# longliangLiu/PriOr-Flow

Measured on AMD Instinct MI355X. Metric: frame-pairs/sec @512x1024 iters=12; EPE vs reference, higher is better.
Workload: dtype bf16x3 split MFMA, f32 accumulate/storage; 1 GPU; PriOr-RAFT forward, 1 synthetic 512x1024 ERP pair(s) per GPU per step, iters=12, test_mode (BASELINE.json configs[1]); height=512, width=1024, iters=12, parallelism=pairs sharded over 1 rank(s), no data-path collective, weights=deterministic closed-form fill (no checkpoints offline), hip_graph=True, encoders=libpriorflow_hip.so (HIP kernels, both precisions)

## Files before the change

### __graft_entry__.py

```python
from __future__ import annotations

import os
import shutil
import subprocess
import sys

ROOT = os.path.dirname(os.path.abspath(__file__))
PKG = os.path.join(ROOT, "prior-flow_amd")
CSRC = os.path.join(PKG, "csrc")
LIB_DIR = os.path.join(PKG, "lib")
LIB = os.path.join(LIB_DIR, "libpriorflow_hip.so")
HIP_UNITS = [("pf_elem_kernels.hip", [], "pf_elem_kernels"), ("pf_lookup.hip", [], "pf_lookup"),
             ("pf_conv_mfma.hip", ["-DPF_CONV_PART=0"], "pf_conv_mfma.p0"), ("pf_conv_mfma.hip", ["-DPF_CONV_PART=1"], "pf_conv_mfma.p1"),
             ("pf_conv_mfma.hip", ["-DPF_CONV_PART=2"], "pf_conv_mfma.p2"), ("pf_conv_mfma.hip", ["-DPF_CONV_PART=3"], "pf_conv_mfma.p3"),
             ("pf_conv_mfma.hip", ["-DPF_CONV_PART=4"], "pf_conv_mfma.p4"),
             ("pf_conv_api.hip", [], "pf_conv_api"),
             ("pf_corr_mfma.hip", [], "pf_corr_mfma"), ("pf_enc_stem.hip", [], "pf_enc_stem"), ("pf_enc_conv.hip", [], "pf_enc_conv"), ("pf_flow_stem.hip", [], "pf_flow_stem"), ("pf_corr_conv.hip", [], "pf_corr_conv"), ("pf_conv_bwd.hip", [], "pf_conv_bwd"),
             ("pf_augment.hip", [], "pf_augment")]
HIP_UNITS += [("pf_conv_dma.hip", [f"-DPF_DMA_PART={i}"], f"pf_conv_dma.p{i}") for i in (0, 1, 2, 3, 4, 5, 6, 7, 8, 9)]
HIP_SOURCES = sorted({u[0] for u in HIP_UNITS})
HIP_DEPS = ["pf_common.h", "pf_elem.h", "pf_split.h", "pf_conv_priv.h", "pf_api_elem.inc", os.path.join("..", "..", "include", "priorflow_hip.h")]
HIPCC_FLAGS = ["--offload-arch=gfx950", "-O3", "-ffp-contract=off", "-fno-slp-vectorize", "-fPIC", "-shared"]


def _stale(target: str, sources) -> bool:
    if not os.path.exists(target):
        return True
    t = os.path.getmtime(target)
    return any(os.path.getmtime(s) > t for s in sources if os.path.exists(s))


def _deps_of(dfile: str, fallback):
    try:
        txt = open(dfile).read().replace("\\\n", " ")
# ... 127 lines not shown
```

### prior-flow_amd/csrc/pf_conv_api.hip

```cpp
#include <stdlib.h>
#include "pf_conv_priv.h"

using namespace pfconv;

static int conv_prepare(const pf_conv_desc* descs, int ngroups, int B, int H8, int W8,
                        ConvGroups& grp, ConvGeom& g, int& max_cout) {
    if (!descs || ngroups < 1 || ngroups > MAX_GROUPS) return PF_ERR_BAD_ARG;
    if (B <= 0 || H8 <= 0 || W8 <= 0) return PF_ERR_BAD_SHAPE;
    max_cout = 0;
    const pf_conv_desc& f = descs[0];
    for (int i = 0; i < ngroups; ++i) {
        const pf_conv_desc& d = descs[i];
        if ((!d.in0 && !d.in0_split) || !d.weight || !d.bias || (!d.out && !d.out_split)) return PF_ERR_BAD_ARG;
        if (d.c0 <= 0 || d.c1 < 0 || (d.c1 > 0 && !d.in1 && !d.in1_split)) return PF_ERR_BAD_ARG;
        const bool f16 = d.precision == PF_PREC_F16;
        const int cpc = f16 ? 64 : 32, cm = cpc - 1;
        if ((d.in0_split || d.in1_split || d.out_split || d.aux_split) && d.precision != PF_PREC_BF16X3 && !f16) return PF_ERR_BAD_ARG;
        if (f16 && (!d.in0_split || (d.c1 > 0 && !d.in1_split))) return PF_ERR_BAD_ARG;
        if (d.in0_split && ((d.off0 & cm) || d.lds0 * cpc < d.off0 + d.c0)) return PF_ERR_BAD_SHAPE;
        if (d.in1_split && d.c1 > 0 && ((d.off1 & cm) || (d.c0 & cm) || d.lds1 * cpc < d.off1 + d.c1)) return PF_ERR_BAD_SHAPE;
        if (d.in0_split && d.c1 == 0 && (d.c0 & cm) && d.off0 + ((d.c0 + cm) & ~cm) != d.lds0 * cpc) return PF_ERR_BAD_SHAPE;
        if (d.in1_split && d.c1 > 0 && (d.c1 & cm) && d.off1 + ((d.c1 + cm) & ~cm) != d.lds1 * cpc) return PF_ERR_BAD_SHAPE;
        if (d.out_split && ((d.off_out & 31) || d.lds_out <= 0)) return PF_ERR_BAD_SHAPE;
        if (d.aux_split && d.lds_aux * cpc < 128) return PF_ERR_BAD_SHAPE;
// ... 58 lines not shown
static bool roles_apply(const ConvGroups& grp, int ngroups, const ConvGeom& g) {
    if (!((g.kh == 3 && g.kw == 3) || (g.kh == 1 && g.kw == 5) || (g.kh == 5 && g.kw == 1)) || g.stride != 1) return false;
    for (int i = 0; i < ngroups; ++i)
        if (grp.d[i].stats_out != nullptr || grp.d[i].in_scale != nullptr) return false;
    return true;
}

static int conv_dma_choice(const ConvGroups& grp, int ngroups, const ConvGeom& g, int max_cout, int tile_id) {
    if (!grp.d[0].in0_split || tile_id < 3 || tile_id == 7 || !roles_apply(grp, ngroups, g)) return 0;
    if (tile_id == 5) return 2;
    const long wgs256 = (long)(g.M / g.N) * ((g.H + 7) / 8) * ((g.W + 31) / 32) * (ngroups + grp.d[0].co_groups) * ((max_cout + 63) / 64);
    if (g.kh != 3 && max_cout > 128 && wgs256 >= 256) return 2;
    return (g.kh == 3 && max_cout > 64 && wgs256 >= 256) ? 2 : 1;
}

static int conv_ws_choice(const ConvGroups& grp, int ngroups, const ConvGeom& g, int max_cout) {
    static const int ws = [] { const char* e = getenv("PRIORFLOW_CONV_WS"); return e ? atoi(e) : 2; }();
    if (ws <= 0 || !roles_apply(grp, ngroups, g)) return 0;
    const long wgs256 = (long)(g.M / g.N) * ((g.H + 7) / 8) * ((g.W + 31) / 32) * ngroups * ((max_cout + 63) / 64);
    if (ws >= 3 && g.kh == 3 && wgs256 >= 256) return 2;
    return (ws >= 2 && g.kh == 3 && max_cout > 64 && wgs256 >= 256) ? 2 : 1;
}

static int conv_plan(const pf_conv_desc* descs, int ngroups, int B, int H8, int W8, ConvPlan& p) {
    if (const int rc = conv_prepare(descs, ngroups, B, H8, W8, p.grp, p.g, p.max_cout)) return rc;
    const ConvGroups& grp = p.grp;
    const ConvGeom& g = p.g;
    p.ngroups = ngroups;
    p.tile = conv_tile(g, ngroups + descs[0].co_groups, p.max_cout, descs[0].precision);
    const int dma = conv_dma_choice(grp, ngroups, g, p.max_cout, p.tile);
    if (descs[0].precision == PF_PREC_F16 && !dma) return PF_ERR_BAD_SHAPE;
    const bool split = descs[0].precision == PF_PREC_BF16X3;
    const bool generic = p.tile < 3 || p.tile == 7;
    const int bm = (p.tile == 0 || p.tile == 7) ? 128 : 64;
    for (int i = 0; i < ngroups; ++i) {
        if (descs[i].in_scale && generic) return PF_ERR_BAD_SHAPE;
        if (descs[i].stats_out && descs[i].epilogue != PF_EPI_LINEAR) return PF_ERR_BAD_SHAPE;
        if (descs[i].stats_out && generic && (!split || g.N % bm != 0)) return PF_ERR_BAD_SHAPE;
    }
    const bool enc64 = (p.tile == 5 || p.tile == 3) && pf_enc_conv64_applies(grp, ngroups, g, p.max_cout);
    const int th = (p.tile == 5 || p.tile == 8) ? 8 : 4;
    p.stats_blocks = enc64 ? pf_enc_conv64_stats_blocks(g)
                   : generic ? ((split && g.N % bm == 0) ? g.N / bm : 0) : ((g.H + th - 1) / th) * ((g.W + 31) / 32);
    p.affine = false;
    if (dma) {
        for (int i = 0; i < ngroups; ++i)
            if (!descs[i].zeros || descs[i].zeros_bytes < 128 * (descs[i].lds0 > descs[i].lds1 ? descs[i].lds0 : descs[i].lds1)) return PF_ERR_BAD_ARG;
        p.roles = 16 + dma;
        p.launch = dma == 2 ? pf_conv_dma_launch<2, 1> : p.tile == 4 ? pf_conv_dma_launch<2, 2> : pf_conv_dma_launch<1, 2>;
        return PF_OK;
    }
    for (int i = 0; i < ngroups; ++i) {
        if (!descs[i].in0 || (descs[i].c1 > 0 && !descs[i].in1)) return PF_ERR_BAD_ARG;
        if (descs[i].pre) return PF_ERR_BAD_SHAPE;
    }
    p.roles = 0;
    if (enc64) { p.tile = 6; p.launch = pf_enc_conv64_launch; return PF_OK; }
    if (!generic) {
        p.affine = descs[0].in_scale != nullptr;
        for (int i = 1; i < ngroups; ++i)
            if ((descs[i].in_scale != nullptr) != p.affine) return PF_ERR_BAD_ARG;
        if (p.affine && (g.kh != 3 || g.kw != 3)) return PF_ERR_BAD_SHAPE;
    }
    if (p.tile == 3 || p.tile == 4) p.roles = conv_ws_choice(grp, ngroups, g, p.max_cout);
// ... 37 lines not shown
```

### prior-flow_amd/csrc/pf_conv_dma.hip

```cpp
#include <stdlib.h>
#include "pf_conv_priv.h"

namespace {
using namespace pfconv;

template <int HP, int HSTEPS>
constexpr int hbeg_(int t) { return t >= HSTEPS ? HP : HP * t / HSTEPS; }

template <int N>
__device__ __forceinline__ void wait_vmcnt() {
#if defined(__HIP_DEVICE_COMPILE__)
    asm volatile("s_waitcnt vmcnt(%0)" :: "n"(N) : "memory");
#endif
}
__device__ __forceinline__ void wg_barrier() {
#if defined(__HIP_DEVICE_COMPILE__) && !defined(PF_DMA_ABL_NO_BARRIER)
    asm volatile("s_barrier" ::: "memory");
#endif
}

struct DmaItem { int grp, tile, ntile; };


typedef _Float16 f16x8 __attribute__((ext_vector_type(8)));

template <int NT, int KH, int KW, int WN, bool F16>
__global__ void __launch_bounds__(512, 2)
pf_conv_dma_kernel(const ConvGroups groups, const ConvGeom g) {
    static_assert(WN == 1 || WN == 2, "");
    constexpr int TH = 8 / WN, TW = 32, BN = 32 * NT * WN, TAPS = KH * KW;
    static_assert(TAPS >= 5, "the halo schedule needs TAPS - 3 >= 2 issue steps");
    constexpr int HW = TW + KW - 1, HH = TH + KH - 1;
    constexpr int HP = (HH * HW + 31) / 32;
    constexpr int HALO_ROWS = 32 * HP, HALO_BYTES = HALO_ROWS * 128;
    constexpr int WP = BN / 32;
    constexpr int SLOT_BYTES = BN * 128;
    constexpr int HSTEPS = TAPS - 3;
    constexpr int CSH = F16 ? 6 : 5;
    extern __shared__ __attribute__((aligned(128))) char smem[];
    constexpr int RING = 2 * HALO_BYTES;

    const int tid = threadIdx.x;
    const int lane = tid & 63, wave = __builtin_amdgcn_readfirstlane(tid >> 6);
    const int li = lane & 31, lh = lane >> 5;
    const int tiles_x = (g.W + TW - 1) / TW, tiles_y = (g.H + TH - 1) / TH;
// ... 151 lines not shown
                        if (ih) wait_vmcnt<hp + WP + hc>();
                        else wait_vmcnt<WP>();
                    } else {
                        wait_vmcnt<0>();
                    }
                    slot3 = (slot3 + 1) & 3;
                });
            }
            have = have_next;
            if (have) have_next = next_item(j, nit);
        }
        return;
    }

    const int wy2 = WN == 2 ? wave >> 1 : wave, wn = WN == 2 ? wave & 1 : 0;
    f32x16 acc[2][NT];
    const unsigned arow0 = (unsigned)((2 * wy2) * HW + li);
    const unsigned P0 = 2u * lh;
    const unsigned b_off = (unsigned)(32 * NT * wn + li) * 128 + ((P0 ^ (((unsigned)(32 * NT * wn + li) >> 1) & 7u)) << 4);
    bf16x8 fa[2][2][4], fb[2][NT][4];
#ifdef PF_DMA_ABL_NO_READS
    for (int i = 0; i < 2; ++i)
        for (int k = 0; k < 4; ++k) {
            for (int m = 0; m < 2; ++m) for (int e = 0; e < 8; ++e) fa[i][m][k][e] = (__bf16)(float)(lane & 7);
            for (int t = 0; t < NT; ++t) for (int e = 0; e < 8; ++e) fb[i][t][k][e] = (__bf16)(float)(lane & 3);
        }
#endif
    unsigned a_addr[2] = {0, 0}, b_addr = 0;
    unsigned a_base[TAPS][2];
    auto set_a_base = [&]() __attribute__((always_inline)) {
        unsigned ar = arow0;
#if defined(__HIP_DEVICE_COMPILE__)
        asm volatile("" : "+v"(ar));
#endif
#pragma unroll
        for (int tp = 0; tp < TAPS; ++tp)
#pragma unroll
            for (int m = 0; m < 2; ++m) {
                const unsigned hr = ar + (unsigned)((tp / KW + m) * HW + tp % KW);
                a_base[tp][m] = (hr << 7) + ((P0 ^ ((hr >> 1) & 7u)) << 4);
            }
    };
    set_a_base();
    constexpr int NP = 8 + 4 * NT;
    constexpr int NM = (F16 ? 8 : 12) * NT;
    constexpr int FETCH_GAPS = NM - 2;
    auto fetch_piece = [&](auto SET, auto P, unsigned halo_off, auto TAP, unsigned slot_off) __attribute__((always_inline)) {
        constexpr int set = decltype(SET)::value, p = decltype(P)::value, tp = decltype(TAP)::value;
        if constexpr (p < 8) {
            constexpr int m = p / 4, k = p % 4;
            if constexpr (k == 0) {
                unsigned a0 = halo_off + a_base[tp][m];
#if defined(__HIP_DEVICE_COMPILE__)
                asm volatile("" : "+v"(a0));
#endif
                a_addr[m] = a0;
            }
            constexpr unsigned x = (k & 1) * 16u + (k >> 1) * 64u;
#ifndef PF_DMA_ABL_NO_READS
            fa[set][m][k] = *reinterpret_cast<const bf16x8*>(smem + (a_addr[m] ^ x));
#endif
        } else {
            constexpr int t = (p - 8) / 4, k = (p - 8) % 4;
            if constexpr (t == 0 && k == 0) b_addr = (unsigned)RING + slot_off + b_off;
            constexpr unsigned x = (k & 1) * 16u + (k >> 1) * 64u;
#ifndef PF_DMA_ABL_NO_READS
            fb[set][t][k] = *reinterpret_cast<const bf16x8*>(smem + (b_addr ^ x) + t * 4096);
#endif
        }
    };
    unsigned jm = wslot;
    DmaItem it;
    if (!next_item(jm, it)) return;
    wg_barrier();
    static_for<0, NP>([&](auto P) __attribute__((always_inline)) { fetch_piece(std::integral_constant<int, 0>{}, P, 0u, std::integral_constant<int, 0>{}, 0u); });
    int slot1 = 1;
    int gc = 0;
    auto mstep = [&](auto U) __attribute__((always_inline)) {
        constexpr int u = decltype(U)::value;
        constexpr int tap = u % TAPS, cur = u & 1;
        constexpr int ntap = (tap + 1) % TAPS;
        const unsigned halo_off = (unsigned)(((tap == TAPS - 1 ? gc + 1 : gc) & 1) * HALO_BYTES), slot_off = (unsigned)(slot1 * SLOT_BYTES);
        using NXT = std::integral_constant<int, cur ^ 1>;
        wg_barrier();
        static_for<0, NM>([&](auto I) __attribute__((always_inline)) {
            constexpr int i = decltype(I)::value;
            constexpr int idx = i % (2 * NT), m = idx / NT, t = idx % NT, j = i / (2 * NT), ks = j / 3, pass = j % 3;
#ifdef PF_DMA_ABL_NO_MFMA
            if constexpr (F16)
                asm volatile("" :: "v"(fa[cur][m][j]), "v"(fb[cur][t][j]));
            else if constexpr (pass == 0)
                asm volatile("" :: "v"(fa[cur][m][ks]), "v"(fa[cur][m][2 + ks]), "v"(fb[cur][t][ks]), "v"(fb[cur][t][2 + ks]));
#else
            if constexpr (F16)
                acc[m][t] = __builtin_amdgcn_mfma_f32_32x32x16_f16(__builtin_bit_cast(f16x8, fa[cur][m][j]),
                                                                  __builtin_bit_cast(f16x8, fb[cur][t][j]), acc[m][t], 0, 0, 0);
            else if constexpr (pass == 0)
                acc[m][t] = __builtin_amdgcn_mfma_f32_32x32x16_bf16(fa[cur][m][2 + ks], fb[cur][t][ks], acc[m][t], 0, 0, 0);
            else if constexpr (pass == 1)
                acc[m][t] = __builtin_amdgcn_mfma_f32_32x32x16_bf16(fa[cur][m][ks], fb[cur][t][2 + ks], acc[m][t], 0, 0, 0);
            else
                acc[m][t] = __builtin_amdgcn_mfma_f32_32x32x16_bf16(fa[cur][m][ks], fb[cur][t][ks], acc[m][t], 0, 0, 0);
// ... 6 lines not shown
        });
        slot1 = (slot1 + 1) & 3;
        if constexpr (tap == TAPS - 1) ++gc;
    };
    const bool ragged = (g.W % TW) != 0 || (g.H % TH) != 0;
    bool have = true;
    while (have) {
        if (const float* pre = gdesc[it.grp].pre) {
            const auto& dp = gdesc[it.grp];
            const int ldp = dp.ld_pre, jb = it.ntile * BN + 32 * NT * wn + li;
            const int cout = dp.cout;
            pre += dp.off_pre;
            int x0, y0; long pix0;
            tile_origin(it, x0, y0, pix0);
#pragma unroll
            for (int m = 0; m < 2; ++m) {
                const int wy = 2 * wy2 + m;
                const int xlim = (y0 + wy < g.H) ? g.W - x0 - 4 * lh : 0;
                const long pm = pix0 + (long)(y0 + wy) * g.W + x0 + 4 * lh;
#pragma unroll
                for (int t = 0; t < NT; ++t) {
                    const bool jok = jb + 32 * t < cout;
                    const float* pp = pre + pm * ldp + jb + 32 * t;
#pragma unroll
                    for (int r = 0; r < 16; ++r) {
                        const int ro = (r & 3) + 8 * (r >> 2);
                        acc[m][t][r] = (jok && ro < xlim) ? pp[(long)ro * ldp] : 0.f;
                    }
                }
            }
        } else {
#pragma unroll
            for (int m = 0; m < 2; ++m)
#pragma unroll
                for (int t = 0; t < NT; ++t)
#pragma unroll
                    for (int r = 0; r < 16; ++r) acc[m][t][r] = 0.f;
        }
        {
            int c2 = 0;
            for (; c2 + 1 < nchunks; c2 += 2)
                static_for<0, 2 * TAPS>([&](auto U) __attribute__((always_inline)) { mstep(U); });
            if (nchunks & 1)
                static_for<0, TAPS>([&](auto U) __attribute__((always_inline)) { mstep(U); });
        }
        const auto& dd = gdesc[it.grp];
        pf_conv_desc d;
        d.bias = dd.bias; d.out = dd.out; d.ld_out = dd.ld_out; d.off_out = dd.off_out; d.cout = dd.cout;
        d.epilogue = dd.epilogue; d.scale = dd.scale; d.h = dd.h; d.ld_h = dd.ld_h; d.z = dd.z; d.ld_z = dd.ld_z;
        d.aux_out = dd.aux_out; d.ld_aux = dd.ld_aux; d.precision = dd.precision;
        d.out_split = dd.out_split; d.lds_out = dd.lds_out; d.aux_split = dd.aux_split; d.lds_aux = dd.lds_aux; d.save_gates = dd.save_gates;
        const int n0 = it.ntile * BN;
        int x0, y0; long pix0;
        tile_origin(it, x0, y0, pix0);
        long p0[2], plim[2];
#pragma unroll
        for (int m = 0; m < 2; ++m) {
            const int wy = 2 * wy2 + m;
            const bool row_ok = y0 + wy < g.H;
            const int xlim = row_ok ? g.W - x0 - 4 * lh : 0;
            p0[m] = pix0 + (long)(y0 + wy) * g.W + x0 + 4 * lh;
            plim[m] = p0[m] + (xlim > 0 ? xlim : 0);
        }
#ifdef PF_DMA_ABL_NO_EPI
#if defined(__HIP_DEVICE_COMPILE__)
        asm volatile("" :: "v"(acc[0][0]), "v"(acc[1][0]), "v"(acc[0][NT - 1]), "v"(acc[1][NT - 1]));
#endif
        (void)d; (void)p0; (void)plim;
#else
        if (ragged) tile_epilogue_pair<NT, true, F16>(d, acc, n0 + 32 * NT * wn, li, p0, plim);
        else tile_epilogue_pair<NT, false, F16>(d, acc, n0 + 32 * NT * wn, li, p0, plim);
#endif
        have = next_item(jm, it);
        if (have) {
            set_a_base();
            const unsigned hoff = (unsigned)((gc & 1) * HALO_BYTES), soff = (unsigned)(((slot1 + 3) & 3) * SLOT_BYTES);
            static_for<0, NP>([&](auto P) __attribute__((always_inline)) { fetch_piece(std::integral_constant<int, 0>{}, P, hoff, std::integral_constant<int, 0>{}, soff); });
        }
    }
}

template <int NT, int KH, int KW, int WN, bool F16>
int launch_conv_dma_t(const ConvGroups& grp, int ngroups, const ConvGeom& g, int max_cout, hipStream_t stream) {
    constexpr int BN = 32 * NT * WN, TH = 8 / WN;
    constexpr int HALO_ROWS = ((TH + KH - 1) * (32 + KW - 1) + 31) / 32 * 32;
    constexpr size_t lds = (size_t)2 * HALO_ROWS * 128 + (size_t)4 * BN * 128;
    static_assert(lds <= 160 * 1024, "LDS budget");
    const int B = g.M / g.N;
    ConvGeom gg = g;
    gg.ntiles = B * ((g.H + TH - 1) / TH) * ((g.W + 31) / 32);
    gg.ntn = (max_cout + BN - 1) / BN;
    gg.xcd_map = 1;
    gg.ngroups = ngroups;
    gg.d_ntn = fd_make((unsigned)gg.ntn); gg.d_ntiles = fd_make((unsigned)gg.ntiles);
    gg.d_tx = fd_make((unsigned)((g.W + 31) / 32)); gg.d_ty = fd_make((unsigned)((g.H + TH - 1) / TH));
    constexpr int MAX_DEV = 64;
    static int cus_of[MAX_DEV];
    static bool attr_set[MAX_DEV];
    int dev = 0;
// ... 8 lines not shown
    if (cap > 0 && cap < 8 && items > cap) cap = 8;
    const dim3 grid((unsigned)((cap > 0 && items > cap) ? cap : items));
    if (!attr_set[dev]) {
        const hipError_t attr = hipFuncSetAttribute(reinterpret_cast<const void*>(&pf_conv_dma_kernel<NT, KH, KW, WN, F16>),
                                                    hipFuncAttributeMaxDynamicSharedMemorySize, 160 * 1024);
        if (attr != hipSuccess) return (int)attr;
        attr_set[dev] = true;
    }
    hipLaunchKernelGGL((pf_conv_dma_kernel<NT, KH, KW, WN, F16>), grid, dim3(512), lds, stream, grp, gg);
    return (int)hipGetLastError();
}

}

#ifndef PF_DMA_PART
#error "compile pf_conv_dma.hip with -DPF_DMA_PART=0..9"
#endif
template <int NT, int KH, int KW, int WN>
int pf_conv_dma_shape_launch(const pfconv::ConvPlan& p, hipStream_t stream);
#if PF_DMA_PART != 7
template <int NT, int KH, int KW, int WN>
int pf_conv_dma_shape_launch(const pfconv::ConvPlan& p, hipStream_t stream) {
    return p.grp.d[0].precision == PF_PREC_F16 ? launch_conv_dma_t<NT, KH, KW, WN, true>(p.grp, p.ngroups, p.g, p.max_cout, stream)
                                               : launch_conv_dma_t<NT, KH, KW, WN, false>(p.grp, p.ngroups, p.g, p.max_cout, stream);
}
#define PF_DMA_SHAPE(NT, KH, KW, WN) template int pf_conv_dma_shape_launch<NT, KH, KW, WN>(const pfconv::ConvPlan&, hipStream_t);
#endif
#if PF_DMA_PART == 0
PF_DMA_SHAPE(2, 3, 3, 1)
#elif PF_DMA_PART == 1
PF_DMA_SHAPE(2, 3, 3, 2)
#elif PF_DMA_PART == 2
PF_DMA_SHAPE(2, 1, 5, 2)
#elif PF_DMA_PART == 3
PF_DMA_SHAPE(2, 5, 1, 2)
#elif PF_DMA_PART == 4
PF_DMA_SHAPE(1, 3, 3, 2)
#elif PF_DMA_PART == 5
PF_DMA_SHAPE(1, 1, 5, 2)
#elif PF_DMA_PART == 6
PF_DMA_SHAPE(1, 5, 1, 2)
#elif PF_DMA_PART == 8
PF_DMA_SHAPE(2, 1, 5, 1)
#elif PF_DMA_PART == 9
PF_DMA_SHAPE(2, 5, 1, 1)
#else
template <int NT, int WN>
int pf_conv_dma_launch(const pfconv::ConvPlan& p, hipStream_t stream) {
    const int kh = p.g.kh, kw = p.g.kw;
    if (kh == 3 && kw == 3) return pf_conv_dma_shape_launch<NT, 3, 3, WN>(p, stream);
    if (kh == 1 && kw == 5) return pf_conv_dma_shape_launch<NT, 1, 5, WN>(p, stream);
    if (kh == 5 && kw == 1) return pf_conv_dma_shape_launch<NT, 5, 1, WN>(p, stream);
    return PF_ERR_BAD_SHAPE;
}
template int pf_conv_dma_launch<2, 1>(const pfconv::ConvPlan&, hipStream_t);
template int pf_conv_dma_launch<2, 2>(const pfconv::ConvPlan&, hipStream_t);
template int pf_conv_dma_launch<1, 2>(const pfconv::ConvPlan&, hipStream_t);
#endif
```

### prior-flow_amd/csrc/pf_conv_priv.h

```cpp
#pragma once
#include <type_traits>
#include "pf_common.h"
#include "../../include/priorflow_hip.h"

namespace pfconv {

typedef float f32x16 __attribute__((ext_vector_type(16)));
typedef float f32x4 __attribute__((ext_vector_type(4)));
typedef __bf16 bf16x4 __attribute__((ext_vector_type(4)));
typedef __bf16 bf16x8 __attribute__((ext_vector_type(8)));

constexpr int KC = 32;
constexpr int LDS_LD = 36;
constexpr int MAX_GROUPS = 4;

struct ConvGroups { pf_conv_desc d[MAX_GROUPS]; };

struct FastDiv { unsigned m, s1, s2; };
inline FastDiv fd_make(unsigned d) {
    FastDiv f{0u, 0u, 0u};
    if (d <= 1) return f;
    unsigned s = 0;
    while ((1ull << s) < d) ++s;
    f.m = (unsigned)((((1ull << 32) * ((1ull << s) - d)) / d) + 1);
// ... 166 lines not shown
#pragma unroll
            for (int r = 0; r < 16; ++r) {
                zv[r] = live(r) ? zp[(long)roff(r) * d.ld_z] : 0.f;
                hv[r] = live(r) ? hp[(long)roff(r) * d.ld_h] : 0.f;
            }
#pragma unroll
            for (int r = 0; r < 16; ++r) v[r] = pf_tanh<FAST>(acc[t][r] + bias);
            if (d.save_gates && d.aux_out != nullptr) put(v, d.aux_out, d.ld_aux, j, nullptr, 0);
#pragma unroll
            for (int r = 0; r < 16; ++r) v[r] = (1.f - zv[r]) * hv[r] + zv[r] * v[r];
            put(v, d.out, d.ld_out, d.off_out + j, d.out_split, d.lds_out);
        }
    }
}

template <int NT, bool CHECK, bool FAST, bool F16OUT = false>
__device__ __forceinline__ void tile_epilogue_pair_t(const pf_conv_desc& d, const f32x16 (&acc)[2][NT], int jb, int li,
                                                     const long (&p0)[2], const long (&plimit)[2]) {
    const int epi = d.epilogue;
    constexpr auto roff = [](int r) constexpr { return (r & 3) + 8 * (r >> 2); };
    float bias[NT];
    f32x16 hv[2][NT], zv[2][NT];
    static_for<0, NT>([&](auto T) __attribute__((always_inline)) {
        constexpr int t = decltype(T)::value;
        const int jt = jb + 32 * t, j = jt + li;
        const bool jok = j < d.cout;
        bias[t] = jok ? d.bias[j] : 0.f;
        const bool need_h = jok && ((epi == PF_EPI_GRU_ZR && jt >= 128) || epi == PF_EPI_GRU_Q || epi == PF_EPI_RELU_RES ||
                                    epi == PF_EPI_MASK || epi == PF_EPI_ADD);
        const bool need_z = jok && epi == PF_EPI_GRU_Q;
        const int hc = epi == PF_EPI_GRU_ZR ? j - 128 : j;
        static_for<0, 2>([&](auto M) __attribute__((always_inline)) {
            constexpr int m = decltype(M)::value;
            if (need_h) {
                const float* hp = d.h + p0[m] * d.ld_h + hc;
                static_for<0, 16>([&](auto R) __attribute__((always_inline)) {
                    constexpr int r = decltype(R)::value;
                    hv[m][t][r] = (!CHECK || p0[m] + roff(r) < plimit[m]) ? hp[(long)roff(r) * d.ld_h] : 0.f;
                });
            }
            if (need_z) {
                const float* zp = d.z + p0[m] * d.ld_z + j;
                static_for<0, 16>([&](auto R) __attribute__((always_inline)) {
                    constexpr int r = decltype(R)::value;
                    zv[m][t][r] = (!CHECK || p0[m] + roff(r) < plimit[m]) ? zp[(long)roff(r) * d.ld_z] : 0.f;
                });
            }
        });
    });
    static_for<0, 2>([&](auto M) __attribute__((always_inline)) {
        constexpr int m = decltype(M)::value;
        const long pm = p0[m], pl = plimit[m];
        auto put = [&](const f32x16& v, float* base, int ld, int col, void* sbase, int lds) __attribute__((always_inline)) {
            if (base != nullptr) {
                float* o = base + pm * ld + col;
                static_for<0, 16>([&](auto R) __attribute__((always_inline)) {
                    constexpr int r = decltype(R)::value;
                    if (!CHECK || pm + roff(r) < pl) o[(long)roff(r) * ld] = v[r];
                });
            }
            if constexpr (F16OUT) {
                if (sbase != nullptr) {
                    char* sp = reinterpret_cast<char*>(sbase) + ((pm * lds + (col >> 6)) * 128 + 2 * (col & 63));
                    const long rs = (long)lds * 128;
                    static_for<0, 16>([&](auto R) __attribute__((always_inline)) {
// ... 51 lines not shown
                    put(v, d.out, d.ld_out, d.off_out + j, d.out_split, d.lds_out);
                } else {
                    static_for<0, 16>([&](auto R) { constexpr int r = decltype(R)::value; v[r] = pf_tanh<FAST>(acc[m][t][r] + b); });
                    if (d.save_gates && d.aux_out != nullptr) put(v, d.aux_out, d.ld_aux, j, nullptr, 0);
                    static_for<0, 16>([&](auto R) {
                        constexpr int r = decltype(R)::value;
                        v[r] = (1.f - zv[m][t][r]) * hv[m][t][r] + zv[m][t][r] * v[r];
                    });
                    put(v, d.out, d.ld_out, d.off_out + j, d.out_split, d.lds_out);
                }
            }
        });
    });
}

template <int NT, bool CHECK, bool F16OUT = false>
__device__ __forceinline__ void tile_epilogue_pair(const pf_conv_desc& d, const f32x16 (&acc)[2][NT], int jb, int li,
                                                   const long (&p0)[2], const long (&plimit)[2]) {
    const bool gated = d.epilogue == PF_EPI_GRU_ZR || d.epilogue == PF_EPI_GRU_Q || d.epilogue == PF_EPI_TANH_RELU;
    if constexpr (F16OUT) tile_epilogue_pair_t<NT, CHECK, true, true>(d, acc, jb, li, p0, plimit);
    else if (gated && d.precision == PF_PREC_F32) tile_epilogue_pair_t<NT, CHECK, false>(d, acc, jb, li, p0, plimit);
    else tile_epilogue_pair_t<NT, CHECK, true>(d, acc, jb, li, p0, plimit);
}

template <int NT, bool CHECK, bool F16OUT = false>
__device__ __forceinline__ void tile_epilogue(const pf_conv_desc& d, const f32x16 (&acc)[NT], int jb, int li,
                                              long p0, long plimit) {
    const bool gated = d.epilogue == PF_EPI_GRU_ZR || d.epilogue == PF_EPI_GRU_Q || d.epilogue == PF_EPI_TANH_RELU;
    if constexpr (F16OUT) tile_epilogue_t<NT, CHECK, true, true>(d, acc, jb, li, p0, plimit);
    else if (gated && d.precision == PF_PREC_F32) tile_epilogue_t<NT, CHECK, false>(d, acc, jb, li, p0, plimit);
    else tile_epilogue_t<NT, CHECK, true>(d, acc, jb, li, p0, plimit);
}

// ... 19 lines not shown
```

### prior-flow_amd/csrc/pf_corr_conv.hip

```cpp
#include <type_traits>
#include "pf_common.h"
#include "pf_elem.h"
#include "pf_split.h"
#include "pf_conv_priv.h"
#include "../../include/priorflow_hip.h"

namespace {

typedef float f32x16 __attribute__((ext_vector_type(16)));
typedef float f32x4 __attribute__((ext_vector_type(4)));
typedef __bf16 bf16x4 __attribute__((ext_vector_type(4)));
typedef __bf16 bf16x8 __attribute__((ext_vector_type(8)));

constexpr int CC_PX = 64;
constexpr int CC_CIN = PF_CORR_CH;
constexpr int CC_NCH = (CC_CIN + 31) / 32;
constexpr int CC_COUT = 256;
constexpr int CC_LDS_A = 2 * CC_PX * 128;
constexpr int CC_LDS = CC_LDS_A + CC_PX * 8 * 4;

struct CombGroups { pf_combine_conv_desc d[2]; int f16; };

template <int I, int N, class F>
__device__ __forceinline__ void cc_for(F&& f) {
// ... 9 lines not shown
    char* const As = cc_smem;
    int* const tap_idx = reinterpret_cast<int*>(cc_smem + CC_LDS_A);
    float* const tap_w = reinterpret_cast<float*>(tap_idx + CC_PX * 4);
    const pf_combine_conv_desc d = blockIdx.y == 0 ? groups.d[0] : groups.d[1];
    const int tid = threadIdx.x;
    const long N = (long)H * W, rows = (long)B * N;
    const long row0 = (long)blockIdx.x * CC_PX;

    const int lane = tid & 63, wave = __builtin_amdgcn_readfirstlane(tid >> 6);
    const int li = lane & 31, lh = lane >> 5;
    const char* wrow[2];
#pragma unroll
    for (int t = 0; t < 2; ++t)
        wrow[t] = reinterpret_cast<const char*>(d.weight) + ((long)(64 * wave + 32 * t + li) * CC_NCH) * 128 + 32 * lh;
    bf16x8 fb[4][2][4];
    auto load_B = [&](auto SLOT, int chunk) __attribute__((always_inline)) {
        constexpr int slot = decltype(SLOT)::value;
#pragma unroll
        for (int t = 0; t < 2; ++t) {
            const char* p = wrow[t] + chunk * 128;
            fb[slot][t][0] = *reinterpret_cast<const bf16x8*>(p);
            fb[slot][t][1] = *reinterpret_cast<const bf16x8*>(p + 16);
            fb[slot][t][2] = *reinterpret_cast<const bf16x8*>(p + 64);
            fb[slot][t][3] = *reinterpret_cast<const bf16x8*>(p + 80);
        }
    };
    load_B(std::integral_constant<int, 0>{}, 0);
    load_B(std::integral_constant<int, 1>{}, 1);
    load_B(std::integral_constant<int, 2>{}, 2);

    if (tid < CC_PX) {
        const long row = row0 + tid;
        PfTaps t;
        if (row < rows) {
            const long n = row % N;
            t = pf_taps0(pf_pymod(d.g_back[n], (float)W), d.g_back[N + n], H, W);
        } else {
            for (int j = 0; j < 4; ++j) { t.idx[j] = 0; t.w[j] = 0.f; }
        }
        for (int j = 0; j < 4; ++j) { tap_idx[tid * 4 + j] = t.idx[j]; tap_w[tid * 4 + j] = t.w[j]; }
    }
    __syncthreads();
    const int kc = tid & 7, px0 = tid >> 3;
    const float* gbase[2][5];
    float gw[2][4];
    bool glive[2];
#pragma unroll
    for (int i = 0; i < 2; ++i) {
        const int px = px0 + 32 * i;
        const long row = row0 + px;
        glive[i] = row < rows;
        const long rr = glive[i] ? row : 0;
        const float* rb = d.raw + (rr / N) * N * d.ld;
#pragma unroll
        for (int j = 0; j < 4; ++j) { gbase[i][j] = rb + (long)tap_idx[px * 4 + j] * d.ld; gw[i][j] = tap_w[px * 4 + j]; }
        gbase[i][4] = d.own + rr * d.ld;
    }
    f32x4 g[2][2][5];
    auto gather = [&](auto SET, int chunk) __attribute__((always_inline)) {
        constexpr int set = decltype(SET)::value;
        const int c = 32 * chunk + 4 * kc;
        const int cc = c < CC_CIN ? c : 0;
#pragma unroll
        for (int i = 0; i < 2; ++i)
#pragma unroll
            for (int j = 0; j < 5; ++j) g[set][i][j] = *reinterpret_cast<const f32x4*>(gbase[i][j] + cc);
    };
    auto combine_to_lds = [&](auto SET, int chunk) __attribute__((always_inline)) {
        constexpr int set = decltype(SET)::value;
        const bool real = 32 * chunk + 4 * kc < CC_CIN;
#pragma unroll
        for (int i = 0; i < 2; ++i) {
            const int px = px0 + 32 * i;
            f32x4 v;
#pragma unroll
            for (int e = 0; e < 4; ++e) {
                float c = g[set][i][0][e] * gw[i][0];
                c = c + g[set][i][1][e] * gw[i][1];
                c = c + g[set][i][2][e] * gw[i][2];
                c = c + g[set][i][3][e] * gw[i][3];
                v[e] = (real && glive[i]) ? g[set][i][4][e] + c : 0.f;
// ... 9 lines not shown
    };
    unsigned a_piece[4];
    {
        const unsigned swz = (unsigned)((li >> 1) & 7), p0 = 2u * lh;
        a_piece[0] = ((p0 + 0) ^ swz) * 16; a_piece[1] = ((p0 + 1) ^ swz) * 16;
        a_piece[2] = ((p0 + 4) ^ swz) * 16; a_piece[3] = ((p0 + 5) ^ swz) * 16;
    }
    const char* const a_lane = As + li * 128;
    f32x16 acc[2][2];
#pragma unroll
    for (int m = 0; m < 2; ++m)
#pragma unroll
        for (int t = 0; t < 2; ++t)
#pragma unroll
            for (int r = 0; r < 16; ++r) acc[m][t][r] = 0.f;
    auto compute = [&](auto SLOT, int chunk) __attribute__((always_inline)) {
        constexpr int slot = decltype(SLOT)::value;
        bf16x8 fa[2][4];
#pragma unroll
        for (int m = 0; m < 2; ++m)
#pragma unroll
            for (int q = 0; q < 4; ++q)
                fa[m][q] = *reinterpret_cast<const bf16x8*>(a_lane + ((chunk & 1) * CC_PX + 32 * m) * 128 + a_piece[q]);
#pragma unroll
        for (int ks = 0; ks < 2; ++ks)
#pragma unroll
            for (int m = 0; m < 2; ++m)
#pragma unroll
                for (int t = 0; t < 2; ++t) {
                    acc[m][t] = __builtin_amdgcn_mfma_f32_32x32x16_bf16(fa[m][2 + ks], fb[slot][t][ks], acc[m][t], 0, 0, 0);
                    acc[m][t] = __builtin_amdgcn_mfma_f32_32x32x16_bf16(fa[m][ks], fb[slot][t][2 + ks], acc[m][t], 0, 0, 0);
                    acc[m][t] = __builtin_amdgcn_mfma_f32_32x32x16_bf16(fa[m][ks], fb[slot][t][ks], acc[m][t], 0, 0, 0);
                }
    };
    gather(std::integral_constant<int, 0>{}, 0);
    gather(std::integral_constant<int, 1>{}, 1);
    cc_for<0, CC_NCH>([&](auto CH) __attribute__((always_inline)) {
        constexpr int chunk = decltype(CH)::value;
        using SET = std::integral_constant<int, chunk & 1>;
        combine_to_lds(SET{}, chunk);
        if constexpr (chunk + 2 < CC_NCH) gather(SET{}, chunk + 2);
        if constexpr (chunk + 3 < CC_NCH) load_B(std::integral_constant<int, (chunk + 3) & 3>{}, chunk + 3);
        __syncthreads();
        compute(std::integral_constant<int, chunk & 3>{}, chunk);
    });
#pragma unroll
    for (int t = 0; t < 2; ++t) {
        const int ch = 64 * wave + 32 * t + li;
        const float bias = d.bias[ch];
#pragma unroll
        for (int m = 0; m < 2; ++m) {
            const long prow = row0 + 32 * m + 4 * lh;
            if (d.out != nullptr) {
                float* o = d.out + prow * d.ld_out + d.off_out + ch;
#pragma unroll
                for (int r = 0; r < 16; ++r) {
                    const int pr = (r & 3) + 8 * (r >> 2);
                    if (prow + pr < rows) o[(long)pr * d.ld_out] = fmaxf(acc[m][t][r] + bias, 0.f);
                }
// ... 49 lines not shown
```

Before: 152.0 frame-pairs/s.

## Add 96-wide single-row-tile DMA conv variant and deepen corr-conv gather pipeline

Adds a new DMA conv kernel instantiation (NT=3, WN=0, one M-row per wave, 4-row tile) for 3x3 stride-1 bf16x3 convolutions whose output channels are a multiple of 96 and above 128. It is selected by default through an environment switch when there are enough tiles, to avoid padding waste on 96-multiple channel counts. Separately, the correlation conv kernel now keeps three gather buffers in flight instead of two and skips MFMA and weight loads for the padded last K-slice. The trade-off is more registers per thread and another compiled unit, which may lower occupancy.

Result: no change. 151.2 frame-pairs/s (-0.6%).

```diff
diff --git a/__graft_entry__.py b/__graft_entry__.py
--- a/__graft_entry__.py
+++ b/__graft_entry__.py
@@ -17,7 +17,7 @@
              ("pf_conv_api.hip", [], "pf_conv_api"),
              ("pf_corr_mfma.hip", [], "pf_corr_mfma"), ("pf_enc_stem.hip", [], "pf_enc_stem"), ("pf_enc_conv.hip", [], "pf_enc_conv"), ("pf_flow_stem.hip", [], "pf_flow_stem"), ("pf_corr_conv.hip", [], "pf_corr_conv"), ("pf_conv_bwd.hip", [], "pf_conv_bwd"),
              ("pf_augment.hip", [], "pf_augment")]
-HIP_UNITS += [("pf_conv_dma.hip", [f"-DPF_DMA_PART={i}"], f"pf_conv_dma.p{i}") for i in (0, 1, 2, 3, 4, 5, 6, 7, 8, 9)]
+HIP_UNITS += [("pf_conv_dma.hip", [f"-DPF_DMA_PART={i}"], f"pf_conv_dma.p{i}") for i in (0, 1, 2, 3, 4, 5, 6, 7, 8, 9, 10)]
 HIP_SOURCES = sorted({u[0] for u in HIP_UNITS})
 HIP_DEPS = ["pf_common.h", "pf_elem.h", "pf_split.h", "pf_conv_priv.h", "pf_api_elem.inc", os.path.join("..", "..", "include", "priorflow_hip.h")]
 HIPCC_FLAGS = ["--offload-arch=gfx950", "-O3", "-ffp-contract=off", "-fno-slp-vectorize", "-fPIC", "-shared"]
diff --git a/prior-flow_amd/csrc/pf_conv_api.hip b/prior-flow_amd/csrc/pf_conv_api.hip
--- a/prior-flow_amd/csrc/pf_conv_api.hip
+++ b/prior-flow_amd/csrc/pf_conv_api.hip
@@ -96,6 +96,15 @@
     return (g.kh == 3 && max_cout > 64 && wgs256 >= 256) ? 2 : 1;
 }
 
+static bool conv_dma96_applies(const ConvGroups& grp, int ngroups, const ConvGeom& g, int max_cout, bool tile4) {
+    static const int sw = [] { const char* e = getenv("PRIORFLOW_CONV_DMA96"); return e ? atoi(e) : 1; }();
+    if (sw <= 0 || ngroups != 1 || g.kh != 3 || g.kw != 3 || g.stride != 1 || grp.d[0].precision != PF_PREC_BF16X3 || !grp.d[0].in0_split) return false;
+    for (int i = 0; i < ngroups; ++i)
+        if (grp.d[i].cout <= 128 || grp.d[i].cout % 96 != 0) return false;
+    const long tiles4 = (long)(g.M / g.N) * ((g.H + 3) / 4) * ((g.W + 31) / 32);
+    return sw >= 2 || (tile4 && tiles4 * (ngroups + grp.d[0].co_groups) * (max_cout / 96) >= 256);
+}
+
 static int conv_ws_choice(const ConvGroups& grp, int ngroups, const ConvGeom& g, int max_cout) {
     static const int ws = [] { const char* e = getenv("PRIORFLOW_CONV_WS"); return e ? atoi(e) : 2; }();
     if (ws <= 0 || !roles_apply(grp, ngroups, g)) return 0;
@@ -110,7 +119,8 @@
     const ConvGeom& g = p.g;
     p.ngroups = ngroups;
     p.tile = conv_tile(g, ngroups + descs[0].co_groups, p.max_cout, descs[0].precision);
-    const int dma = conv_dma_choice(grp, ngroups, g, p.max_cout, p.tile);
+    int dma = conv_dma_choice(grp, ngroups, g, p.max_cout, p.tile);
+    if (dma && conv_dma96_applies(grp, ngroups, g, p.max_cout, dma == 1 && p.tile == 4)) { dma = 3; p.tile = 4; }
     if (descs[0].precision == PF_PREC_F16 && !dma) return PF_ERR_BAD_SHAPE;
     const bool split = descs[0].precision == PF_PREC_BF16X3;
     const bool generic = p.tile < 3 || p.tile == 7;
@@ -129,7 +139,7 @@
         for (int i = 0; i < ngroups; ++i)
             if (!descs[i].zeros || descs[i].zeros_bytes < 128 * (descs[i].lds0 > descs[i].lds1 ? descs[i].lds0 : descs[i].lds1)) return PF_ERR_BAD_ARG;
         p.roles = 16 + dma;
-        p.launch = dma == 2 ? pf_conv_dma_launch<2, 1> : p.tile == 4 ? pf_conv_dma_launch<2, 2> : pf_conv_dma_launch<1, 2>;
+        p.launch = dma == 3 ? pf_conv_dma_launch<3, 0> : dma == 2 ? pf_conv_dma_launch<2, 1> : p.tile == 4 ? pf_conv_dma_launch<2, 2> : pf_conv_dma_launch<1, 2>;
         return PF_OK;
     }
     for (int i = 0; i < ngroups; ++i) {
diff --git a/prior-flow_amd/csrc/pf_conv_dma.hip b/prior-flow_amd/csrc/pf_conv_dma.hip
--- a/prior-flow_amd/csrc/pf_conv_dma.hip
+++ b/prior-flow_amd/csrc/pf_conv_dma.hip
@@ -27,8 +27,10 @@
 template <int NT, int KH, int KW, int WN, bool F16>
 __global__ void __launch_bounds__(512, 2)
 pf_conv_dma_kernel(const ConvGroups groups, const ConvGeom g) {
-    static_assert(WN == 1 || WN == 2, "");
-    constexpr int TH = 8 / WN, TW = 32, BN = 32 * NT * WN, TAPS = KH * KW;
+    static_assert(WN == 0 || WN == 1 || WN == 2, "");
+    constexpr int MR = WN == 0 ? 1 : 2;
+    constexpr int WNC = WN == 0 ? 1 : WN;
+    constexpr int TH = 4 * MR / WNC, TW = 32, BN = 32 * NT * WNC, TAPS = KH * KW;
     static_assert(TAPS >= 5, "the halo schedule needs TAPS - 3 >= 2 issue steps");
     constexpr int HW = TW + KW - 1, HH = TH + KH - 1;
     constexpr int HP = (HH * HW + 31) / 32;
@@ -210,20 +212,20 @@
     }
 
     const int wy2 = WN == 2 ? wave >> 1 : wave, wn = WN == 2 ? wave & 1 : 0;
-    f32x16 acc[2][NT];
-    const unsigned arow0 = (unsigned)((2 * wy2) * HW + li);
+    f32x16 acc[MR][NT];
+    const unsigned arow0 = (unsigned)((MR * wy2) * HW + li);
     const unsigned P0 = 2u * lh;
     const unsigned b_off = (unsigned)(32 * NT * wn + li) * 128 + ((P0 ^ (((unsigned)(32 * NT * wn + li) >> 1) & 7u)) << 4);
-    bf16x8 fa[2][2][4], fb[2][NT][4];
+    bf16x8 fa[2][MR][4], fb[2][NT][4];
 #ifdef PF_DMA_ABL_NO_READS
     for (int i = 0; i < 2; ++i)
         for (int k = 0; k < 4; ++k) {
-            for (int m = 0; m < 2; ++m) for (int e = 0; e < 8; ++e) fa[i][m][k][e] = (__bf16)(float)(lane & 7);
+            for (int m = 0; m < MR; ++m) for (int e = 0; e < 8; ++e) fa[i][m][k][e] = (__bf16)(float)(lane & 7);
             for (int t = 0; t < NT; ++t) for (int e = 0; e < 8; ++e) fb[i][t][k][e] = (__bf16)(float)(lane & 3);
         }
 #endif
-    unsigned a_addr[2] = {0, 0}, b_addr = 0;
-    unsigned a_base[TAPS][2];
+    unsigned a_addr[MR] = {}, b_addr = 0;
+    unsigned a_base[TAPS][MR];
     auto set_a_base = [&]() __attribute__((always_inline)) {
         unsigned ar = arow0;
 #if defined(__HIP_DEVICE_COMPILE__)
@@ -232,18 +234,18 @@
 #pragma unroll
         for (int tp = 0; tp < TAPS; ++tp)
 #pragma unroll
-            for (int m = 0; m < 2; ++m) {
+            for (int m = 0; m < MR; ++m) {
                 const unsigned hr = ar + (unsigned)((tp / KW + m) * HW + tp % KW);
                 a_base[tp][m] = (hr << 7) + ((P0 ^ ((hr >> 1) & 7u)) << 4);
             }
     };
     set_a_base();
-    constexpr int NP = 8 + 4 * NT;
-    constexpr int NM = (F16 ? 8 : 12) * NT;
+    constexpr int NP = 4 * MR + 4 * NT;
+    constexpr int NM = (F16 ? 4 : 6) * MR * NT;
     constexpr int FETCH_GAPS = NM - 2;
     auto fetch_piece = [&](auto SET, auto P, unsigned halo_off, auto TAP, unsigned slot_off) __attribute__((always_inline)) {
         constexpr int set = decltype(SET)::value, p = decltype(P)::value, tp = decltype(TAP)::value;
-        if constexpr (p < 8) {
+        if constexpr (p < 4 * MR) {
             constexpr int m = p / 4, k = p % 4;
             if constexpr (k == 0) {
                 unsigned a0 = halo_off + a_base[tp][m];
@@ -257,7 +259,7 @@
             fa[set][m][k] = *reinterpret_cast<const bf16x8*>(smem + (a_addr[m] ^ x));
 #endif
         } else {
-            constexpr int t = (p - 8) / 4, k = (p - 8) % 4;
+            constexpr int t = (p - 4 * MR) / 4, k = (p - 4 * MR) % 4;
             if constexpr (t == 0 && k == 0) b_addr = (unsigned)RING + slot_off + b_off;
             constexpr unsigned x = (k & 1) * 16u + (k >> 1) * 64u;
 #ifndef PF_DMA_ABL_NO_READS
@@ -281,7 +283,7 @@
         wg_barrier();
         static_for<0, NM>([&](auto I) __attribute__((always_inline)) {
             constexpr int i = decltype(I)::value;
-            constexpr int idx = i % (2 * NT), m = idx / NT, t = idx % NT, j = i / (2 * NT), ks = j / 3, pass = j % 3;
+            constexpr int idx = i % (MR * NT), m = idx / NT, t = idx % NT, j = i / (MR * NT), ks = j / 3, pass = j % 3;
 #ifdef PF_DMA_ABL_NO_MFMA
             if constexpr (F16)
                 asm volatile("" :: "v"(fa[cur][m][j]), "v"(fb[cur][t][j]));
@@ -318,8 +320,8 @@
             int x0, y0; long pix0;
             tile_origin(it, x0, y0, pix0);
 #pragma unroll
-            for (int m = 0; m < 2; ++m) {
-                const int wy = 2 * wy2 + m;
+            for (int m = 0; m < MR; ++m) {
+                const int wy = MR * wy2 + m;
                 const int xlim = (y0 + wy < g.H) ? g.W - x0 - 4 * lh : 0;
                 const long pm = pix0 + (long)(y0 + wy) * g.W + x0 + 4 * lh;
 #pragma unroll
@@ -335,7 +337,7 @@
             }
         } else {
 #pragma unroll
-            for (int m = 0; m < 2; ++m)
+            for (int m = 0; m < MR; ++m)
 #pragma unroll
                 for (int t = 0; t < NT; ++t)
 #pragma unroll
@@ -357,10 +359,10 @@
         const int n0 = it.ntile * BN;
         int x0, y0; long pix0;
         tile_origin(it, x0, y0, pix0);
-        long p0[2], plim[2];
-#pragma unroll
-        for (int m = 0; m < 2; ++m) {
-            const int wy = 2 * wy2 + m;
+        long p0[MR], plim[MR];
+#pragma unroll
+        for (int m = 0; m < MR; ++m) {
+            const int wy = MR * wy2 + m;
             const bool row_ok = y0 + wy < g.H;
             const int xlim = row_ok ? g.W - x0 - 4 * lh : 0;
             p0[m] = pix0 + (long)(y0 + wy) * g.W + x0 + 4 * lh;
@@ -368,7 +370,7 @@
         }
 #ifdef PF_DMA_ABL_NO_EPI
 #if defined(__HIP_DEVICE_COMPILE__)
-        asm volatile("" :: "v"(acc[0][0]), "v"(acc[1][0]), "v"(acc[0][NT - 1]), "v"(acc[1][NT - 1]));
+        asm volatile("" :: "v"(acc[0][0]), "v"(acc[MR - 1][0]), "v"(acc[0][NT - 1]), "v"(acc[MR - 1][NT - 1]));
 #endif
         (void)d; (void)p0; (void)plim;
 #else
@@ -386,7 +388,7 @@
 
 template <int NT, int KH, int KW, int WN, bool F16>
 int launch_conv_dma_t(const ConvGroups& grp, int ngroups, const ConvGeom& g, int max_cout, hipStream_t stream) {
-    constexpr int BN = 32 * NT * WN, TH = 8 / WN;
+    constexpr int BN = WN == 0 ? 32 * NT : 32 * NT * WN, TH = WN == 0 ? 4 : 8 / WN;
     constexpr int HALO_ROWS = ((TH + KH - 1) * (32 + KW - 1) + 31) / 32 * 32;
     constexpr size_t lds = (size_t)2 * HALO_ROWS * 128 + (size_t)4 * BN * 128;
     static_assert(lds <= 160 * 1024, "LDS budget");
@@ -425,14 +427,17 @@
 }
 
 #ifndef PF_DMA_PART
-#error "compile pf_conv_dma.hip with -DPF_DMA_PART=0..9"
+#error "compile pf_conv_dma.hip with -DPF_DMA_PART=0..10"
 #endif
 template <int NT, int KH, int KW, int WN>
 int pf_conv_dma_shape_launch(const pfconv::ConvPlan& p, hipStream_t stream);
 #if PF_DMA_PART != 7
 template <int NT, int KH, int KW, int WN>
 int pf_conv_dma_shape_launch(const pfconv::ConvPlan& p, hipStream_t stream) {
-    return p.grp.d[0].precision == PF_PREC_F16 ? launch_conv_dma_t<NT, KH, KW, WN, true>(p.grp, p.ngroups, p.g, p.max_cout, stream)
+    if constexpr (WN == 0)
+        return p.grp.d[0].precision == PF_PREC_F16 ? (int)PF_ERR_BAD_SHAPE : launch_conv_dma_t<NT, KH, KW, WN, false>(p.grp, p.ngroups, p.g, p.max_cout, stream);
+    else
+        return p.grp.d[0].precision == PF_PREC_F16 ? launch_conv_dma_t<NT, KH, KW, WN, true>(p.grp, p.ngroups, p.g, p.max_cout, stream)
                                                : launch_conv_dma_t<NT, KH, KW, WN, false>(p.grp, p.ngroups, p.g, p.max_cout, stream);
 }
 #define PF_DMA_SHAPE(NT, KH, KW, WN) template int pf_conv_dma_shape_launch<NT, KH, KW, WN>(const pfconv::ConvPlan&, hipStream_t);
@@ -455,6 +460,8 @@
 PF_DMA_SHAPE(2, 1, 5, 1)
 #elif PF_DMA_PART == 9
 PF_DMA_SHAPE(2, 5, 1, 1)
+#elif PF_DMA_PART == 10
+PF_DMA_SHAPE(3, 3, 3, 0)
 #else
 template <int NT, int WN>
 int pf_conv_dma_launch(const pfconv::ConvPlan& p, hipStream_t stream) {
@@ -464,6 +471,10 @@
     if (kh == 5 && kw == 1) return pf_conv_dma_shape_launch<NT, 5, 1, WN>(p, stream);
     return PF_ERR_BAD_SHAPE;
 }
+template <>
+int pf_conv_dma_launch<3, 0>(const pfconv::ConvPlan& p, hipStream_t stream) {
+    return (p.g.kh == 3 && p.g.kw == 3) ? pf_conv_dma_shape_launch<3, 3, 3, 0>(p, stream) : (int)PF_ERR_BAD_SHAPE;
+}
 template int pf_conv_dma_launch<2, 1>(const pfconv::ConvPlan&, hipStream_t);
 template int pf_conv_dma_launch<2, 2>(const pfconv::ConvPlan&, hipStream_t);
 template int pf_conv_dma_launch<1, 2>(const pfconv::ConvPlan&, hipStream_t);
diff --git a/prior-flow_amd/csrc/pf_conv_priv.h b/prior-flow_amd/csrc/pf_conv_priv.h
--- a/prior-flow_amd/csrc/pf_conv_priv.h
+++ b/prior-flow_amd/csrc/pf_conv_priv.h
@@ -204,13 +204,13 @@
     }
 }
 
-template <int NT, bool CHECK, bool FAST, bool F16OUT = false>
-__device__ __forceinline__ void tile_epilogue_pair_t(const pf_conv_desc& d, const f32x16 (&acc)[2][NT], int jb, int li,
-                                                     const long (&p0)[2], const long (&plimit)[2]) {
+template <int NT, bool CHECK, bool FAST, bool F16OUT = false, int MR>
+__device__ __forceinline__ void tile_epilogue_pair_t(const pf_conv_desc& d, const f32x16 (&acc)[MR][NT], int jb, int li,
+                                                     const long (&p0)[MR], const long (&plimit)[MR]) {
     const int epi = d.epilogue;
     constexpr auto roff = [](int r) constexpr { return (r & 3) + 8 * (r >> 2); };
     float bias[NT];
-    f32x16 hv[2][NT], zv[2][NT];
+    f32x16 hv[MR][NT], zv[MR][NT];
     static_for<0, NT>([&](auto T) __attribute__((always_inline)) {
         constexpr int t = decltype(T)::value;
         const int jt = jb + 32 * t, j = jt + li;
@@ -220,7 +220,7 @@
                                     epi == PF_EPI_MASK || epi == PF_EPI_ADD);
         const bool need_z = jok && epi == PF_EPI_GRU_Q;
         const int hc = epi == PF_EPI_GRU_ZR ? j - 128 : j;
-        static_for<0, 2>([&](auto M) __attribute__((always_inline)) {
+        static_for<0, MR>([&](auto M) __attribute__((always_inline)) {
             constexpr int m = decltype(M)::value;
             if (need_h) {
                 const float* hp = d.h + p0[m] * d.ld_h + hc;
@@ -238,7 +238,7 @@
             }
         });
     });
-    static_for<0, 2>([&](auto M) __attribute__((always_inline)) {
+    static_for<0, MR>([&](auto M) __attribute__((always_inline)) {
         constexpr int m = decltype(M)::value;
         const long pm = p0[m], pl = plimit[m];
         auto put = [&](const f32x16& v, float* base, int ld, int col, void* sbase, int lds) __attribute__((always_inline)) {
@@ -320,9 +320,9 @@
     });
 }
 
-template <int NT, bool CHECK, bool F16OUT = false>
-__device__ __forceinline__ void tile_epilogue_pair(const pf_conv_desc& d, const f32x16 (&acc)[2][NT], int jb, int li,
-                                                   const long (&p0)[2], const long (&plimit)[2]) {
+template <int NT, bool CHECK, bool F16OUT = false, int MR>
+__device__ __forceinline__ void tile_epilogue_pair(const pf_conv_desc& d, const f32x16 (&acc)[MR][NT], int jb, int li,
+                                                   const long (&p0)[MR], const long (&plimit)[MR]) {
     const bool gated = d.epilogue == PF_EPI_GRU_ZR || d.epilogue == PF_EPI_GRU_Q || d.epilogue == PF_EPI_TANH_RELU;
     if constexpr (F16OUT) tile_epilogue_pair_t<NT, CHECK, true, true>(d, acc, jb, li, p0, plimit);
     else if (gated && d.precision == PF_PREC_F32) tile_epilogue_pair_t<NT, CHECK, false>(d, acc, jb, li, p0, plimit);
diff --git a/prior-flow_amd/csrc/pf_corr_conv.hip b/prior-flow_amd/csrc/pf_corr_conv.hip
--- a/prior-flow_amd/csrc/pf_corr_conv.hip
+++ b/prior-flow_amd/csrc/pf_corr_conv.hip
@@ -47,20 +47,24 @@
     for (int t = 0; t < 2; ++t)
         wrow[t] = reinterpret_cast<const char*>(d.weight) + ((long)(64 * wave + 32 * t + li) * CC_NCH) * 128 + 32 * lh;
     bf16x8 fb[4][2][4];
-    auto load_B = [&](auto SLOT, int chunk) __attribute__((always_inline)) {
-        constexpr int slot = decltype(SLOT)::value;
+    constexpr int CC_KS_LAST = (CC_CIN - 32 * (CC_NCH - 1) + 15) / 16;
+    auto load_B = [&](auto SLOT, auto CH) __attribute__((always_inline)) {
+        constexpr int slot = decltype(SLOT)::value, chunk = decltype(CH)::value;
+        constexpr int nks = chunk == CC_NCH - 1 ? CC_KS_LAST : 2;
 #pragma unroll
         for (int t = 0; t < 2; ++t) {
             const char* p = wrow[t] + chunk * 128;
             fb[slot][t][0] = *reinterpret_cast<const bf16x8*>(p);
-            fb[slot][t][1] = *reinterpret_cast<const bf16x8*>(p + 16);
             fb[slot][t][2] = *reinterpret_cast<const bf16x8*>(p + 64);
-            fb[slot][t][3] = *reinterpret_cast<const bf16x8*>(p + 80);
-        }
-    };
-    load_B(std::integral_constant<int, 0>{}, 0);
-    load_B(std::integral_constant<int, 1>{}, 1);
-    load_B(std::integral_constant<int, 2>{}, 2);
+            if constexpr (nks > 1) {
+                fb[slot][t][1] = *reinterpret_cast<const bf16x8*>(p + 16);
+                fb[slot][t][3] = *reinterpret_cast<const bf16x8*>(p + 80);
+            }
+        }
+    };
+    load_B(std::integral_constant<int, 0>{}, std::integral_constant<int, 0>{});
+    load_B(std::integral_constant<int, 1>{}, std::integral_constant<int, 1>{});
+    load_B(std::integral_constant<int, 2>{}, std::integral_constant<int, 2>{});
 
     if (tid < CC_PX) {
         const long row = row0 + tid;
@@ -89,15 +93,16 @@
         for (int j = 0; j < 4; ++j) { gbase[i][j] = rb + (long)tap_idx[px * 4 + j] * d.ld; gw[i][j] = tap_w[px * 4 + j]; }
         gbase[i][4] = d.own + rr * d.ld;
     }
-    f32x4 g[2][2][5];
-    auto gather = [&](auto SET, int chunk) __attribute__((always_inline)) {
-        constexpr int set = decltype(SET)::value;
+    f32x4 g[3][2][5];
+    auto gather = [&](auto SET, auto CH) __attribute__((always_inline)) {
+        constexpr int set = decltype(SET)::value, chunk = decltype(CH)::value;
         const int c = 32 * chunk + 4 * kc;
-        const int cc = c < CC_CIN ? c : 0;
-#pragma unroll
-        for (int i = 0; i < 2; ++i)
-#pragma unroll
-            for (int j = 0; j < 5; ++j) g[set][i][j] = *reinterpret_cast<const f32x4*>(gbase[i][j] + cc);
+        if (32 * chunk + 32 <= CC_CIN || c < CC_CIN) {
+#pragma unroll
+            for (int i = 0; i < 2; ++i)
+#pragma unroll
+                for (int j = 0; j < 5; ++j) g[set][i][j] = *reinterpret_cast<const f32x4*>(gbase[i][j] + c);
+        }
     };
     auto combine_to_lds = [&](auto SET, int chunk) __attribute__((always_inline)) {
         constexpr int set = decltype(SET)::value;
@@ -137,16 +142,17 @@
         for (int t = 0; t < 2; ++t)
 #pragma unroll
             for (int r = 0; r < 16; ++r) acc[m][t][r] = 0.f;
-    auto compute = [&](auto SLOT, int chunk) __attribute__((always_inline)) {
-        constexpr int slot = decltype(SLOT)::value;
+    auto compute = [&](auto SLOT, auto CH) __attribute__((always_inline)) {
+        constexpr int slot = decltype(SLOT)::value, chunk = decltype(CH)::value;
+        constexpr int nks = chunk == CC_NCH - 1 ? CC_KS_LAST : 2;
         bf16x8 fa[2][4];
 #pragma unroll
         for (int m = 0; m < 2; ++m)
 #pragma unroll
             for (int q = 0; q < 4; ++q)
-                fa[m][q] = *reinterpret_cast<const bf16x8*>(a_lane + ((chunk & 1) * CC_PX + 32 * m) * 128 + a_piece[q]);
-#pragma unroll
-        for (int ks = 0; ks < 2; ++ks)
+                if ((q & 1) < nks) fa[m][q] = *reinterpret_cast<const bf16x8*>(a_lane + ((chunk & 1) * CC_PX + 32 * m) * 128 + a_piece[q]);
+#pragma unroll
+        for (int ks = 0; ks < nks; ++ks)
 #pragma unroll
             for (int m = 0; m < 2; ++m)
 #pragma unroll
@@ -156,16 +162,20 @@
                     acc[m][t] = __builtin_amdgcn_mfma_f32_32x32x16_bf16(fa[m][ks], fb[slot][t][ks], acc[m][t], 0, 0, 0);
                 }
     };
-    gather(std::integral_constant<int, 0>{}, 0);
-    gather(std::integral_constant<int, 1>{}, 1);
+    gather(std::integral_constant<int, 0>{}, std::integral_constant<int, 0>{});
+    gather(std::integral_constant<int, 1>{}, std::integral_constant<int, 1>{});
+    gather(std::integral_constant<int, 2>{}, std::integral_constant<int, 2>{});
     cc_for<0, CC_NCH>([&](auto CH) __attribute__((always_inline)) {
         constexpr int chunk = decltype(CH)::value;
-        using SET = std::integral_constant<int, chunk & 1>;
+        using SET = std::integral_constant<int, chunk % 3>;
+        using NEXT = std::integral_constant<int, chunk + 3>;
         combine_to_lds(SET{}, chunk);
-        if constexpr (chunk + 2 < CC_NCH) gather(SET{}, chunk + 2);
-        if constexpr (chunk + 3 < CC_NCH) load_B(std::integral_constant<int, (chunk + 3) & 3>{}, chunk + 3);
+        if constexpr (chunk + 3 < CC_NCH) {
+            gather(SET{}, NEXT{});
+            load_B(std::integral_constant<int, (chunk + 3) & 3>{}, NEXT{});
+        }
         __syncthreads();
-        compute(std::integral_constant<int, chunk & 3>{}, chunk);
+        compute(std::integral_constant<int, chunk & 3>{}, CH);
     });
 #pragma unroll
     for (int t = 0; t < 2; ++t) {
```
